# liangheming/simple_pose

Hardware: AMD Instinct MI355X
Metric: images/sec fwd+decode, ResNet50-DConv 256x192 bs=128 (higher is better)
Workload: dtype f32; 1 GPU; ResNet50-DConv 256x192 bs=128 per GPU, fp32 forward (NCHW in -> heat maps) + GaussTaylor decode, eval-mode BN, conditioned random weights; images_per_gpu=128, global_batch=128, parallelism=replicas x1 (no collective), ranks=1 process(es), one per GPU, launch=stream launches, tile_table=profiles/r06_dconv_f32_tiles.json, batches_in_flight=2, decode=in line, HSA_ENABLE_IPC_MODE_LEGACY=0

## Files before the change

### include/simple_pose_hip.h

```cpp
#ifndef SIMPLE_POSE_HIP_H
#define SIMPLE_POSE_HIP_H

#include <stdint.h>

#ifdef __cplusplus
extern "C" {
#endif

#define SP_OK 0
#define SP_EINVAL (-1)
#define SP_ELAUNCH (-2)

#define SP_ABI_VERSION 36

#define SP_CONV_RELU 0x1u
#define SP_CONV_OUT_NCHW 0x2u
#define SP_CONV_PIXEL_SHUFFLE 0x4u
#define SP_CONV_OUT_F32 0x10u
#define SP_CONV_BN_Y_MASK 0x20u
#define SP_CONV_BF16 0x8u
#define SP_CONV_HARDSWISH 0x40u
#define SP_CONV_OUT_SLICE 0x80u

typedef struct sp_conv_desc {
    int32_t batch, in_h, in_w, c_in;
    int32_t grid_h, grid_w;
    int32_t c_out;
    int32_t n_pad;
    int32_t taps_h, taps_w;
    int32_t k_pad;
    int32_t stride;
    int32_t dy0, dy_step, dx0, dx_step;
    int32_t out_h, out_w, out_c;
    int32_t oy_mul, oy_add, ox_mul, ox_add;
    int32_t phases_y, phases_x;
    uint32_t flags;
    int32_t tile_m, tile_n;
    int32_t stride_x;
    int32_t kernel;
    int32_t c_in_group;
} sp_conv_desc;

#define SP_CONV_KERNEL_IGEMM 0
#define SP_CONV_KERNEL_RING 1
#define SP_CONV_KERNEL_RING_LW 3
#define SP_CONV_KERNEL_RING_LW4 4
#define SP_CONV_KERNEL_PW 2

int sp_abi_version(void);
const char* sp_last_error(void);


int sp_nchw_to_nhwc4(const float* x_nchw, float* y_nhwc4, int batch, int channels, int h, int w, void* stream);

int sp_conv2d_fwd(const sp_conv_desc* desc, const void* x, const void* w_packed, const float* scale,
                  const float* shift, const void* residual, void* y, void* stream);

int sp_conv_set_tap_skip(int on);

int sp_conv3x3_direct_ok(const sp_conv_desc* desc);
int sp_conv3x3_direct(const sp_conv_desc* desc, const void* x, const void* w_packed, const float* scale, const float* shift,
                      const void* residual, void* y, void* stream);

int sp_basic_block_c32_ok(const sp_conv_desc* desc);
int sp_basic_block_c32(const sp_conv_desc* desc, const void* x, const void* w1_packed, const float* scale1, const float* shift1,
                       const void* w2_packed, const float* scale2, const float* shift2, void* y, void* stream);

int sp_basic_block_c64_ok(const sp_conv_desc* desc);
int sp_basic_block_c64(const sp_conv_desc* desc, const void* x, const void* w1_packed, const float* scale1, const float* shift1,
                       const void* w2_packed, const float* scale2, const float* shift2, void* y, void* stream);

int sp_dual_pw_bf16_ok(int64_t rows, int c_main, int c_short, int c_out);
int sp_dual_pw_f32_ok(int64_t rows, int c_main, int c_short, int c_out);
int sp_dual_pw_f32(const float* a_main, const float* w_main_packed, const float* scale_main, const float* shift_main, const float* a_short,
                   const float* w_short_packed, const float* scale_short, const float* shift_short, float* y, int64_t rows, int c_main, int c_short,
                   int c_out, int relu, void* stream);
int sp_dual_pw_bf16(const void* a_main, const void* w_main_packed, const float* scale_main, const float* shift_main, const void* a_short,
                    const void* w_short_packed, const float* scale_short, const float* shift_short, void* y, int64_t rows, int c_main, int c_short,
                    int c_out, int relu, void* stream);
int sp_pw_chain_f32_ok(int64_t rows, int c_mid, int c_out, int c_next);
int sp_pw_chain_f32(const float* t, const float* w3_packed, const float* scale3, const float* shift3, const float* residual, float* y,
                    const float* w1_packed, const float* scale1, const float* shift1, float* t_next, int64_t rows, int c_mid, int c_out, int c_next,
                    void* stream);
int sp_bottleneck_c64_ok(const sp_conv_desc* desc);
int sp_bottleneck_c64(const sp_conv_desc* desc, const void* x, const void* w1_packed, const float* scale1, const float* shift1,
                      const void* w2_packed, const float* scale2, const float* shift2, const void* w3_packed, const float* scale3,
                      const float* shift3, void* y, void* stream);

int sp_stem7_pool_ok(int batch, int h, int w);
int sp_stem7_pool(const float* x, const void* w_packed, int k_pad, const float* scale, const float* shift, void* y, int bf16,
                  int batch, int h, int w, void* stream);
int sp_stem7_pool_u8(const unsigned char* crops_bgr, const float* mean_rgb_host, const void* w_packed, int k_pad, const float* scale,
                     const float* shift, void* y, int bf16, int batch, int h, int w, void* stream);

int sp_hrnet_transition1_ok(int c_in, int h, int w);
int sp_hrnet_transition1(const void* x, int batch, int h, int w, const void* wa_packed, int k_pad, const float* scale_a, const float* shift_a,
                         const void* wb_packed, const float* scale_b, const float* shift_b, void* y_hi, void* y_lo, void* stream);
int sp_hrnet_stem_ok(int batch, int h, int w);
int sp_hrnet_stem(const float* x, const void* w1_packed, int k1_pad, const float* scale1, const float* shift1, const void* w2_packed,
                  const float* scale2, const float* shift2, void* y, int batch, int h, int w, void* stream);

int sp_conv2d_pw_ok(const sp_conv_desc* desc);

int sp_conv2d_ring_ok(const sp_conv_desc* desc);

int sp_conv2d_kernel_name(const sp_conv_desc* desc, int has_residual, int variant, char* buf, int cap);

int sp_conv2d_default_tile(const sp_conv_desc* desc, int* tile_m, int* tile_n);

int sp_maxpool3x3s2_nhwc(const float* x, float* y, int batch, int h, int w, int c, void* stream);

int sp_pixel_shuffle2_nhwc(const float* x, float* y, int batch, int h, int w, int c, void* stream);

int sp_global_avg_pool_nhwc(const float* x, float* y, int batch, int hw, int c, void* stream);
int sp_se_gate_add_relu_nhwc(const float* x, const float* gate_logits, const float* identity, float* y, int batch, int hw,
                             int c, void* stream);

int sp_upsample_add_nhwc(const float* x, const float* base, float* y, int batch, int h, int w, int c, int factor, int relu,
                         void* stream);
int sp_upsample_add_n_nhwc(const void* base, int bf16, int n_terms, const void* const* xs, const int32_t* factors, void* y, int batch,
                           int out_h, int out_w, int c, int relu, void* stream);

int sp_nchw_to_nhwc8_bf16(const float* x_nchw, void* y_nhwc8, int batch, int channels, int h, int w, void* stream);
int sp_maxpool3x3s2_nhwc_bf16(const void* x, void* y, int batch, int h, int w, int c, void* stream);
int sp_pixel_shuffle2_nhwc_bf16(const void* x, void* y, int batch, int h, int w, int c, void* stream);
int sp_upsample_add_nhwc_bf16(const void* x, const void* base, void* y, int batch, int h, int w, int c, int factor,
                              int relu, void* stream);
int sp_global_avg_pool_nhwc_bf16(const void* x, void* y, int batch, int hw, int c, void* stream);
int sp_se_gate_add_relu_nhwc_bf16(const void* x, const void* gate_logits, const void* identity, void* y, int batch, int hw,
                                  int c, void* stream);


int sp_heat_map_to_axis(const float* heat_nchw, int batch, int joints, int h, int w, float* coords, float* max_val,
                        void* stream);
int sp_decode_gauss_taylor(const float* heat_nchw, const float* trans_inv, int batch, int joints, int h, int w,
                           int kernel_size, float* kps, float* max_val, void* stream);
int sp_decode_basic(const float* heat_nchw, const float* trans_inv, int batch, int joints, int h, int w, float* kps,
                    float* max_val, void* stream);

int sp_heat_map_acc(const float* pred_coords, const float* label_coords, const float* mask, int batch, int joints, int h, int w,
                    float distance_thresh, float norm_frac, float* acc_out, void* stream);

int sp_u8hwc_bgr_to_nchw_f32(const unsigned char* img, float* out, int batch, int h, int w, const float* mean_rgb_host,
                             void* stream);

int sp_warp_affine_u8c3(const unsigned char* src, int src_h, int src_w, const double* m_fwd, int crops, unsigned char* dst, int out_h,
                        int out_w, void* stream);
int sp_warp_affine_batch_u8c3_to_nchw_f32(const unsigned char* const* srcs, const int* src_hw, const int* flip, const double* m_fwd, int batch,
                                          int out_h, int out_w, const float* mean_rgb_host, float* out, unsigned char* crops, void* stream);

int sp_pose_score(const float* max_val, int batch, int joints, float* score, void* stream);
int sp_pose_rescore(const float* kps, const double* box_score, int persons, int joints, double in_vis_thre, double* kps64,
                    double* score, void* stream);
int sp_oks_nms(const double* kps, const double* scores, const double* areas, const int32_t* seg, int groups, int max_group,
               int joints, const double* sigmas_host, double thresh, double vis_thresh, int32_t* keep, int32_t* keep_count,
               void* stream);

#define SP_COCO_MAX_JOINTS 64
#define SP_COCO_MAX_GT_PER_IMAGE 128
#define SP_COCO_MAX_DT_PER_IMAGE 2048
#define SP_COCO_MAX_DETS 32
#define SP_COCO_MAX_THRS 16
#define SP_COCO_MAX_AREAS 4
#define SP_COCO_MAX_REC_THRS 128
#define SP_COCO_DT_XY_F64 1
#define SP_COCO_DT_SCORE_F64 2
// ... 332 lines not shown
```

### simple_pose_amd/_lib.py

```python
from __future__ import annotations

import ctypes
import os
from ctypes import c_double, c_float, c_int, c_int32, c_int64, c_uint32, c_void_p

from .build import LIB_PATH as _DEFAULT_LIB_PATH

LIB_PATH = os.environ.get("SIMPLE_POSE_HIP_LIB", _DEFAULT_LIB_PATH)

SP_CONV_RELU = 0x1
SP_CONV_OUT_NCHW = 0x2
SP_CONV_PIXEL_SHUFFLE = 0x4
SP_CONV_BF16 = 0x8
SP_CONV_OUT_F32 = 0x10
SP_CONV_BN_Y_MASK = 0x20
SP_CONV_HARDSWISH = 0x40
SP_CONV_OUT_SLICE = 0x80
SP_LETTERBOX_FOCUS, SP_LETTERBOX_U8 = 0, 1
SP_YOLO_NMS_MAX_CANDIDATES, SP_YOLO_NMS_MAX_DET = 32768, 1024
SP_COCO_MAX_JOINTS, SP_COCO_MAX_GT_PER_IMAGE, SP_COCO_MAX_DT_PER_IMAGE, SP_COCO_MAX_DETS = 64, 128, 2048, 32
SP_COCO_DT_XY_F64, SP_COCO_DT_SCORE_F64, SP_COCO_GT_CROWD, SP_COCO_GT_IGNORE = 1, 2, 1, 2
CONV_TILES =((128, 128), (64, 128), (128, 64), (64, 64), (256, 64), (128, 32))
ABI_VERSION = 36
SP_CONV_KERNEL_IGEMM, SP_CONV_KERNEL_RING, SP_CONV_KERNEL_PW, SP_CONV_KERNEL_RING_LW, SP_CONV_KERNEL_RING_LW4 = 0, 1, 2, 3, 4
# ... 95 lines not shown
    "sp_decode_basic": (c_int, [_P, _P, c_int, c_int, c_int, c_int, _P, _P, _P]),
    "sp_heat_map_acc": (c_int, [_P, _P, _P, c_int, c_int, c_int, c_int, c_float, c_float, _P, _P]),
    "sp_u8hwc_bgr_to_nchw_f32": (c_int, [_P, _P, c_int, c_int, c_int, ctypes.POINTER(c_float), _P]),
    "sp_encode_gauss_refine": (c_int, [_P, c_int, c_int, c_int, c_int, c_float, _P, _P, _P]),
    "sp_encode_gauss_basic": (c_int, [_P, c_int, c_int, c_int, c_int, c_float, c_int, _P, _P, _P]),
    "sp_bn_train_stats_nhwc": (c_int, [_P, c_int, c_int64, c_int, c_float, c_float, _P, _P, _P, _P, _P, _P]),
    "sp_bn_apply_maxpool_nhwc": (c_int, [_P, c_int, _P, _P, _P, _P, _P, _P, c_int, c_int, c_int, c_int, _P]),
    "sp_bn_maxpool_bwd_nhwc": (c_int, [_P, c_int, _P, _P, _P, _P, _P, _P, c_int, c_int, c_int, c_int, _P, _P, _P, _P, _P]),
    "sp_bn_apply_nhwc": (c_int, [_P, c_int, _P, _P, _P, _P, _P, _P, c_int64, c_int, c_int, _P, _P]),
    "sp_bn_train_partial_nhwc": (c_int, [_P, c_int, c_int64, c_int, _P, _P, _P]),
    "sp_bn_train_finalize": (c_int, [_P, c_int64, c_int, c_float, c_float, _P, _P, _P, _P, _P]),
    "sp_bn_apply_sums_nhwc": (c_int, [_P, c_int, _P, c_int64, c_float, c_float, _P, _P, _P, _P, c_int64, c_int, c_int, _P, _P, _P, _P, _P]),
    "sp_bn_bwd_sums_from_conv2": (c_int, [_P, _P, c_int, c_int, c_int, _P, _P, _P, _P, _P]),
    "sp_bn_train_bwd_reduce_nhwc": (c_int, [_P, c_int, _P, _P, _P, _P, c_int64, c_int, _P, _P, _P, _P]),
    "sp_bn_train_bwd_apply_nhwc": (c_int, [_P, c_int, _P, _P, _P, _P, _P, _P, _P, c_int64, c_int64, c_int, _P, _P, c_int, _P]),
    "sp_bn_train_bwd_nhwc": (c_int, [_P, c_int, _P, _P, _P, _P, _P, c_int64, c_int, _P, _P, _P, _P, c_int, _P, _P]),
    "sp_channel_sum_nchw": (c_int, [_P, c_int, c_int, c_int, _P, _P]),
    "sp_channel_sum_nhwc": (c_int, [_P, c_int64, c_int, _P, _P, _P]),
    "sp_maxpool3x3s2_bwd_nhwc": (c_int, [_P, c_int, _P, _P, c_int, c_int, c_int, c_int, _P]),
    "sp_adam_step": (c_int, [_P, _P, _P, _P, c_int64, c_double, c_double, c_double, c_double, c_int, c_float, _P]),
    "sp_upsample_add_bwd_nhwc": (c_int, [_P, c_int, _P, c_int, c_int, c_int, c_int, c_int, _P, c_int, _P, c_int, _P]),
    "sp_se_gate_bwd_reduce": (c_int, [_P, c_int, _P, _P, c_int, c_int, c_int, _P, _P]),
    "sp_se_sigmoid_bwd": (c_int, [_P, c_int, _P, c_int, c_int, _P, _P, _P]),
    "sp_relu_bwd_rows": (c_int, [_P, c_int, _P, c_int, c_int, _P, _P, _P]),
    "sp_se_gate_bwd_apply": (c_int, [_P, c_int, _P, _P, _P, c_int, c_int, c_int, _P, _P, c_int, _P]),
    "sp_adam_set_scalars": (c_int, [c_double, c_double, c_double, c_double, c_int, c_float, _P, _P]),
    "sp_adam_step_dev": (c_int, [_P, _P, _P, _P, c_int64, _P, _P]),
    "sp_upsample_add_n_nhwc": (c_int, [_P, c_int, c_int, ctypes.POINTER(ctypes.c_void_p), ctypes.POINTER(c_int32), _P, c_int, c_int, c_int, c_int, c_int, _P]),
    "sp_comm_available": (c_int, []),
    "sp_comm_unique_id": (c_int, [_P]),
    "sp_comm_create": (c_int, [_P, c_int, c_int, ctypes.POINTER(ctypes.c_void_p)]),
    "sp_comm_allreduce_sum_f32": (c_int, [_P, _P, c_int64, _P]),
    "sp_comm_allreduce_sum_f64": (c_int, [_P, _P, c_int64, _P]),
    "sp_comm_info": (c_int, [_P, ctypes.POINTER(c_int), ctypes.POINTER(c_int), ctypes.POINTER(c_int)]),
    "sp_comm_destroy": (c_int, [_P]),
    "sp_conv2d_wgrad": (c_int, [ctypes.POINTER(ConvDesc), _P, c_int, _P, c_int, c_int, c_int, c_int64, c_int64, _P, _P, c_int64, _P]),
    "sp_conv2d_wgrad_workspace": (c_int, [ctypes.POINTER(WgradJob), c_int, ctypes.POINTER(c_int64)]),
    "sp_conv2d_wgrad_batched": (c_int, [ctypes.POINTER(WgradJob), c_int, _P, c_int64, _P]),
    "sp_stream_delay_us": (c_int, [c_double, _P]),
    "sp_permute4_f32": (c_int, [_P, _P, c_int, ctypes.POINTER(c_int32), ctypes.POINTER(c_int64), ctypes.POINTER(c_int32), c_int64, c_int64, _P]),
    "sp_permute4_batched": (c_int, [_P, _P, c_int, c_int, _P]),
    "sp_permute4_batched_tiled": (c_int, [_P, _P, c_int, c_int, _P]),
    "sp_pose_score": (c_int, [_P, c_int, c_int, _P, _P]),
    "sp_pose_rescore": (c_int, [_P, _P, c_int, c_int, c_double, _P, _P, _P]),
    "sp_oks_nms": (c_int, [_P, _P, _P, _P, c_int, c_int, c_int, _P, c_double, c_double, _P, _P, _P]),
    "sp_coco_kp_eval_images": (c_int, [_P, _P, _P, _P, _P, _P, _P, _P, _P, c_int, c_int, c_int, c_int, c_int, c_int, ctypes.POINTER(c_double), c_int,
                                       ctypes.POINTER(c_double), c_int, ctypes.POINTER(c_double), c_int, _P, _P, _P, _P, _P, _P, _P, _P, _P]),
    "sp_coco_kp_accumulate_workspace": (c_int, [c_int, c_int, c_int, c_int, ctypes.POINTER(c_int64)]),
    "sp_coco_kp_accumulate": (c_int, [_P, _P, _P, _P, _P, c_int, c_int, c_int, c_int, c_int, ctypes.POINTER(c_double), c_int, _P, c_int64, _P, _P, _P]),
    "sp_pixel_unshuffle2_nhwc": (c_int, [_P, _P, c_int, c_int, c_int, c_int, _P]),
    "sp_pixel_unshuffle2_nhwc_bf16": (c_int, [_P, _P, c_int, c_int, c_int, c_int, _P]),
    "sp_maxpool3x3s2_idx_nhwc": (c_int, [_P, c_int, _P, _P, c_int, c_int, c_int, c_int, _P]),
    "sp_maxpool3x3s2_bwd_idx_nhwc": (c_int, [_P, _P, c_int, _P, c_int, c_int, c_int, c_int, _P]),
    "sp_nchw_to_nhwc_pad": (c_int, [_P, _P, c_int, c_int, c_int, c_int, c_int, c_int, _P]),
    "sp_warp_affine_u8c3": (c_int, [_P, c_int, c_int, _P, c_int, _P, c_int, c_int, _P]),
    "sp_warp_affine_batch_u8c3_to_nchw_f32": (c_int, [_P, _P, _P, _P, c_int, c_int, c_int, ctypes.POINTER(c_float), _P, _P, _P]),
    "sp_conv2d_bn_stats_rows": (c_int, [ctypes.POINTER(ConvDesc), ctypes.POINTER(c_int)]),
    "sp_conv2d_fwd_bn_stats": (c_int, [ctypes.POINTER(ConvDesc), _P, _P, _P, _P, _P, c_int, _P]),
    "sp_conv2d_fwd_bn_stats_abn": (c_int, [ctypes.POINTER(ConvDesc), _P, _P, _P, _P, _P, _P, _P, _P, _P, _P, _P, c_int, _P]),
    "sp_bn_train_stats_from_conv": (c_int, [_P, _P, c_int, c_int, c_int64, c_int, c_float, c_float, _P, _P, _P, _P, _P]),
    "sp_conv2d_dgrad_bn_bwd_stats": (c_int, [ctypes.POINTER(ConvDesc), _P, _P, _P, _P, _P, _P, _P, _P, _P, _P, c_int, _P]),
    "sp_conv2d_dgrad_bn_bwd_stats2": (c_int, [ctypes.POINTER(ConvDesc), _P, _P, _P, _P, _P, _P, _P, _P, _P, _P, _P, _P, _P, _P, c_int, _P]),
    "sp_conv2d_dgrad_bn_bwd_stats_macc": (c_int, [ctypes.POINTER(ConvDesc), _P, _P, _P, _P, _P, _P, _P, _P, _P, _P, _P, _P, _P, _P, _P, c_int, _P]),
    "sp_conv2d_dgrad_phases": (c_int, [ctypes.POINTER(ConvDesc), c_int, _P, ctypes.POINTER(_P), _P, _P, _P, _P, _P, _P, _P, _P, _P, _P, _P, _P, c_int, _P]),
    "sp_bn_sums_from_conv": (c_int, [_P, _P, c_int, c_int, c_int, _P, _P]),
    "sp_bn_fold_apply_nhwc": (c_int, [_P, c_int, _P, _P, c_int, c_int, c_int64, c_float, c_float, _P, _P, _P, _P, c_int64, c_int, c_int, _P, _P, _P, _P, _P, _P]),
    "sp_bn_fold_bwd_apply_nhwc": (c_int, [_P, c_int, _P, _P, _P, _P, _P, c_int, c_int, _P, _P, _P, c_int64, c_int64, c_int, _P, _P, _P, _P, _P, _P, c_int, _P]),
    "sp_bn_bwd_sums_from_conv": (c_int, [_P, _P, c_int, c_int, c_int, _P, _P, _P]),
    "sp_bn_bwd_sums_from_conv_pair": (c_int, [_P, _P, _P, c_int, c_int, c_int, _P, _P, _P, _P, _P]),
    "sp_u8hwc_bgr_to_nhwc": (c_int, [_P, _P, c_int, c_int, c_int, c_int, _P, _P]),
    "sp_nchw_to_nhwc4_bf16": (c_int, [_P, _P, c_int, c_int, c_int, c_int, _P]),
    "sp_conv3x3_direct_ok": (c_int, [ctypes.POINTER(ConvDesc)]),
    "sp_conv3x3_direct": (c_int, [ctypes.POINTER(ConvDesc), _P, _P, _P, _P, _P, _P, _P]),
    "sp_basic_block_c32_ok": (c_int, [ctypes.POINTER(ConvDesc)]),
    "sp_basic_block_c32": (c_int, [ctypes.POINTER(ConvDesc), _P, _P, _P, _P, _P, _P, _P, _P, _P]),
    "sp_basic_block_c64_ok": (c_int, [ctypes.POINTER(ConvDesc)]),
    "sp_basic_block_c64": (c_int, [ctypes.POINTER(ConvDesc), _P, _P, _P, _P, _P, _P, _P, _P, _P]),
    "sp_dual_pw_bf16_ok": (c_int, [c_int64, c_int, c_int, c_int]),
    "sp_dual_pw_f32_ok": (c_int, [c_int64, c_int, c_int, c_int]),
    "sp_dual_pw_f32": (c_int, [_P, _P, _P, _P, _P, _P, _P, _P, _P, c_int64, c_int, c_int, c_int, c_int, _P]),
    "sp_dual_pw_bf16": (c_int, [_P, _P, _P, _P, _P, _P, _P, _P, _P, c_int64, c_int, c_int, c_int, c_int, _P]),
    "sp_pw_chain_f32_ok": (c_int, [c_int64, c_int, c_int, c_int]),
    "sp_pw_chain_f32": (c_int, [_P, _P, _P, _P, _P, _P, _P, _P, _P, _P, c_int64, c_int, c_int, c_int, _P]),
    "sp_bottleneck_c64_ok": (c_int, [ctypes.POINTER(ConvDesc)]),
    "sp_conv2d_pw_ok": (c_int, [ctypes.POINTER(ConvDesc)]),
    "sp_hrnet_stem_ok": (c_int, [c_int, c_int, c_int]),
    "sp_hrnet_stem": (c_int, [_P, _P, c_int, _P, _P, _P, _P, _P, _P, c_int, c_int, c_int, _P]),
    "sp_hrnet_transition1_ok": (c_int, [c_int, c_int, c_int]),
    "sp_hrnet_transition1": (c_int, [_P, c_int, c_int, c_int, _P, c_int, _P, _P, _P, _P, _P, _P, _P, _P]),
    "sp_stem7_pool_ok": (c_int, [c_int, c_int, c_int]),
    "sp_stem7_pool": (c_int, [_P, _P, c_int, _P, _P, _P, c_int, c_int, c_int, c_int, _P]),
    "sp_stem7_pool_u8": (c_int, [_P, ctypes.POINTER(ctypes.c_float), _P, c_int, _P, _P, _P, c_int, c_int, c_int, c_int, _P]),
    "sp_bottleneck_c64": (c_int, [ctypes.POINTER(ConvDesc), _P, _P, _P, _P, _P, _P, _P, _P, _P, _P, _P, _P]),
    "sp_masked_mse": (c_int, [_P, _P, _P, c_int, c_int, c_int, _P, _P, _P, _P]),
    "sp_conv_packed_dims": (c_int, [c_int, c_int, c_int, ctypes.POINTER(c_int), ctypes.POINTER(c_int)]),
    "sp_pack_conv_weights": (c_int, [_P, c_int, c_int, c_int, c_int, c_int, c_int, c_int, c_int, c_int, c_int, _P, c_int, _P]),
    "sp_pack_conv_weights_grouped": (c_int, [_P, c_int, c_int, c_int, c_int, c_int, _P, c_int, _P]),
    "sp_pack_conv_weights_grouped_taps": (c_int, [_P, c_int, c_int, c_int, c_int, c_int, c_int, c_int, c_int, c_int, c_int, c_int, c_int, _P, c_int, _P]),
    "sp_conv2d_wgrad_grouped_workspace": (c_int, [c_int, c_int, c_int, c_int, c_int, c_int, ctypes.POINTER(c_int64)]),
    "sp_conv2d_wgrad_grouped": (c_int, [_P, _P, c_int, c_int, c_int, c_int, c_int, c_int, c_int, c_int, c_int, c_int, c_int, c_int, _P, _P, c_int64, _P]),
    "sp_pack_deconv_k4s2p1": (c_int, [_P, c_int, c_int, c_int, _P, c_int, _P]),
    "sp_fold_bn": (c_int, [_P, _P, _P, _P, c_int, c_float, c_int, _P, _P, _P]),
    "sp_yolo_letterbox": (c_int, [_P, c_int, c_int, c_int, c_int, c_int, c_int, c_int, c_int, c_int, c_int, _P, _P]),
    "sp_yolo_focus_nchw": (c_int, [_P, c_int, c_int, c_int, _P, _P]),
    "sp_yolo_spp_nhwc": (c_int, [_P, c_int, c_int, c_int, c_int, c_int, _P]),
    "sp_upsample2_slice_nhwc": (c_int, [_P, c_int, _P, c_int, c_int, c_int, c_int, c_int, _P]),
    "sp_yolo_head_decode": (c_int, [_P, _P, _P, c_int, ctypes.POINTER(c_int32), c_int, c_int, c_int, ctypes.POINTER(c_float), ctypes.POINTER(c_float), _P, _P]),
    "sp_yolo_nms_workspace": (c_int, [c_int, ctypes.POINTER(c_int64)]),
    "sp_yolo_nms": (c_int, [_P, c_int, c_int, c_int, c_float, c_float, c_int, c_int, c_int, c_int, _P, c_int64, _P, ctypes.POINTER(c_int32), ctypes.POINTER(c_int32), _P]),
    "sp_yolo_boxes_to_source": (c_int, [_P, c_int, c_float, c_float, c_float, c_float, c_float, _P]),
    "sp_yolo_nms_device": (c_int, [_P, c_int, c_int, c_int, c_float, c_float, c_int, c_int, c_int, c_int, _P, c_int64, _P, _P, _P, _P]),
    "sp_topdown_plan": (c_int, [_P, _P, c_int, c_int, c_int, c_float, c_int, c_int, c_int, c_int, c_int, _P, _P, _P, _P, _P, _P, _P, _P, _P, _P, _P]),
    "sp_warp_affine_plan_u8c3": (c_int, [_P, c_int, c_int, c_int, _P, _P, _P, c_int, _P, c_int, c_int, _P]),
    "sp_mirror_w": (c_int, [_P, _P, c_int64, c_int, c_int, _P]),
    "sp_heat_map_flip_merge": (c_int, [_P, _P, ctypes.POINTER(c_int32), c_int, c_int, c_int, c_int, c_int, _P, _P]),
    "sp_track_associate": (c_int, [_P, _P, _P, _P, _P, _P, c_int, c_int, ctypes.POINTER(c_double), c_double, c_int, c_int, _P, _P, _P, _P, _P, _P, _P, _P,
                                   _P, _P]),
    "sp_track_boxes": (c_int, [_P, _P, _P, _P, c_int, c_int, c_float, c_float, c_float, c_int, c_int, c_int, _P, _P, _P]),
    "sp_jpeg_parse": (c_int, [_P, c_int64, ctypes.POINTER(JpegDesc), _P, c_int32]),
    "sp_jpeg_decode_batch": (c_int, [_P, _P, c_int, _P, c_int64, _P, c_int64, _P, c_int64, _P, c_int64, _P, c_int64, _P, c_int, _P]),
    "sp_jpeg_parse_scans": (c_int, [_P, c_int64, ctypes.POINTER(JpegDesc), _P, c_int32, ctypes.POINTER(c_int32), _P, c_int32]),
    "sp_jpeg_progressive_entropy": (c_int, [_P, _P, c_int, _P, _P, _P, _P, c_int64, _P, c_int64, _P, c_int64, _P, c_int64, _P, _P]),
    "sp_jpeg_enc_plan": (c_int, [c_int, c_int, c_int, c_int, c_int, ctypes.POINTER(JpegEncDesc)]),
    "sp_jpeg_encode_batch": (c_int, [_P, _P, c_int, _P, c_int64, _P, c_int64, _P, _P, c_int, _P]),
    "sp_render_workspace_bytes": (c_int, [c_int, c_int, c_int, ctypes.POINTER(c_int64)]),
    "sp_render_poses_u8c3": (c_int, [_P, _P, c_int, c_int, _P, _P, _P, _P, _P, _P, c_int, c_int, c_int, ctypes.POINTER(RenderStyle), _P, _P]),
}

_lib = None


def lib():
    global _lib
    if _lib is None:
        if not os.path.isfile(LIB_PATH):
            raise HipLibraryError(
                f"{LIB_PATH} is missing: build it with `python -m simple_pose_amd.build` (hipcc, gfx950). "
                "simple_pose_amd has no CPU/torch fallback.")
        import torch

        handle = ctypes.CDLL(LIB_PATH)
        for name, (res, args) in SYMBOLS.items():
            fn = getattr(handle, name)
            fn.restype, fn.argtypes = res, args
        if handle.sp_abi_version() != ABI_VERSION:
            raise HipLibraryError(f"ABI mismatch: library {handle.sp_abi_version()} vs binding {ABI_VERSION}")
        _lib = handle
    return _lib


def conv_kernel_name(desc, has_residual: bool = False, variant: int = 0) -> str:
    buf = ctypes.create_string_buffer(256)
    check(lib().sp_conv2d_kernel_name(desc, int(has_residual), variant, buf, 256), "sp_conv2d_kernel_name")
    return buf.value.decode()


def check(rc: int, what: str = ""):
    if rc != 0:
        msg = lib().sp_last_error().decode("utf-8", "replace")
        err = HipLibraryError(f"{what or 'libsimple_pose_hip'} failed (code {rc}): {msg}")
        err.code = rc
        raise err


def ptr(t):
    return None if t is None else t.data_ptr()
# ... 58 lines not shown
```

### simple_pose_amd/csrc/conv_pw.hip

```cpp
#include "sp_common.h"

namespace {

struct PwArgs {
    const float* x;
    const float* w;
    const float* scale;
    const float* shift;
    const float* res;
    float* y;
    int M, N, nchunks, tiles_m, relu;
    unsigned x_bytes, y_bytes;
};

constexpr int BM = 64;
constexpr int TRS = 68;
constexpr unsigned OOB = 0x80000000u;

template <int K>
__global__ __launch_bounds__(256, 1) void conv_pw_kernel(const PwArgs p) {
    constexpr int CH = K / 4;
    constexpr int NG = K / 8;
    constexpr int APT = BM * CH / 256;
    extern __shared__ __align__(16) float smem[];
// ... 353 lines not shown
        const float* a = As + cur * (BM * K);
        f32x4 fa[2][2];
#pragma unroll
        for (int i = 0; i < 2; ++i) fa[0][i] = *reinterpret_cast<const f32x4*>(a + swz(i * 32 + fr, fh));
#pragma unroll
        for (int g = 0; g < NG; ++g) {
            if (g + 1 < NG) {
#pragma unroll
                for (int i = 0; i < 2; ++i) fa[(g + 1) & 1][i] = *reinterpret_cast<const f32x4*>(a + swz(i * 32 + fr, 2 * (g + 1) + fh));
            }
#pragma unroll
            for (int s = 0; s < 4; ++s)
#pragma unroll
                for (int i = 0; i < 2; ++i)
#pragma unroll
                    for (int n = 0; n < 2; ++n)
                        acc[i][n] = __builtin_amdgcn_mfma_f32_32x32x2f32(fa[g & 1][i][s], fb[g][n][s], acc[i][n], 0, 0, 0);
        }

#pragma unroll
        for (int i = 0; i < 2; ++i)
#pragma unroll
            for (int n = 0; n < 2; ++n)
#pragma unroll
                for (int r = 0; r < 16; ++r) tr[(i * 32 + (r & 3) + 8 * (r >> 2) + 4 * fh) * TRS + n * 32 + fr] = acc[i][n][r];
#pragma unroll
        for (int it = 0; it < 16; ++it) {
            f32x4* const slot4 = reinterpret_cast<f32x4*>(tr + (it * 4 + rsub) * TRS + c4);
            f32x4 v = *slot4;
#pragma unroll
            for (int e = 0; e < 4; ++e) v[e] = v[e] * sc4[e] + sh4[e];
            const f32x4 r4 = __builtin_bit_cast(f32x4, rv[it]);
#pragma unroll
            for (int e = 0; e < 4; ++e) v[e] += r4[e];
#pragma unroll
            for (int e = 0; e < 4; ++e) v[e] = v[e] > 0.f ? v[e] : 0.f;
            __builtin_amdgcn_raw_buffer_store_b128(__builtin_bit_cast(u32x4, v), yr, off[it], 0, 0);
            *slot4 = v;
        }
        if (more) park_a(cur ^ 1);
        __syncthreads();
        if (more) load_res(mt + nslots);

        f32x16 c[RT];
#pragma unroll
        for (int i = 0; i < RT; ++i)
#pragma unroll
            for (int r = 0; r < 16; ++r) c[i][r] = 0.f;
        auto yfrag = [&](int i, int g) { return *reinterpret_cast<const f32x4*>(ys + (g >> 3) * (BM * TRS) + ((ri0 + i) * 32 + fr) * TRS + 8 * (g & 7) + 4 * fh); };
        f32x4 fy[2][RT];
#pragma unroll
        for (int i = 0; i < RT; ++i) fy[0][i] = yfrag(i, 0);
#pragma unroll
        for (int g = 0; g < NG1; ++g) {
            if (g + 1 < NG1) {
#pragma unroll
                for (int i = 0; i < RT; ++i) fy[(g + 1) & 1][i] = yfrag(i, g + 1);
            }
#pragma unroll
            for (int s = 0; s < 4; ++s)
#pragma unroll
                for (int i = 0; i < RT; ++i) c[i] = __builtin_amdgcn_mfma_f32_32x32x2f32(fy[g & 1][i][s], fw[g][s], c[i], 0, 0, 0);
        }
#pragma unroll
        for (int i = 0; i < RT; ++i)
#pragma unroll
            for (int r = 0; r < 16; ++r) {
                float v = c[i][r] * s1v + h1v;
                v = v > 0.f ? v : 0.f;
                t2[(i * 32 + (r & 3) + 8 * (r >> 2) + 4 * fh) * T2S + fr] = v;
            }
#pragma unroll
        for (int it = 0; it < RT * 4; ++it) {
            const int lr = it * 8 + (lane >> 3), cc = (lane & 7) * 4;
            const int row = m0 + ri0 * 32 + lr;
            const unsigned o = row < p.M ? (unsigned)(((size_t)row * NEXT + cn * 32 + cc) * 4) : OOB;
            const f32x4 v = *reinterpret_cast<const f32x4*>(t2 + lr * T2S + cc);
            __builtin_amdgcn_raw_buffer_store_b128(__builtin_bit_cast(u32x4, v), tnr, o, 0, 0);
        }
        __syncthreads();
    }
}

template <int NEXT>
int launch_pw_chain(const PwChainArgs& a, hipStream_t stream) {
    constexpr int lds = (2 * BM * 64 + 4 * BM * TRS + 4 * (NEXT / 64) * 32 * T2S) * 4;
    if (sp_reserve_lds<&conv_pw_chain_kernel<64, NEXT>>(lds, "conv_pw_chain")) return SP_ELAUNCH;
    int slots = sp_device_cus();
    if (slots < 1) slots = 1;
    if (slots > a.tiles_m) slots = a.tiles_m;
    const int rounds = (a.tiles_m + slots - 1) / slots;
    slots = (a.tiles_m + rounds - 1) / rounds;
    hipLaunchKernelGGL((conv_pw_chain_kernel<64, NEXT>), dim3(slots), dim3(256), lds, stream, a);
    return sp_check_launch("conv_pw_chain_kernel");
}

template <int K>
int launch_pw_dual(const PwDualArgs& a, hipStream_t stream) {
    constexpr int lds = (4 * BM * K + 4 * BM * TRS) * 4;
    if (sp_reserve_lds<&conv_pw_dual_kernel<K>>(lds, "conv_pw_dual")) return SP_ELAUNCH;
    int slots = sp_device_cus() / a.nchunks;
    if (slots < 1) slots = 1;
    if (slots > a.tiles_m) slots = a.tiles_m;
    const int rounds = (a.tiles_m + slots - 1) / slots;
    slots = (a.tiles_m + rounds - 1) / rounds;
    hipLaunchKernelGGL(conv_pw_dual_kernel<K>, dim3(slots * a.nchunks), dim3(256), lds, stream, a);
    return sp_check_launch("conv_pw_dual_kernel");
}

template <int K>
int launch_pw(const PwArgs& a, hipStream_t stream) {
    constexpr int lds = (2 * BM * K + 4 * BM * TRS) * 4;
    if (sp_reserve_lds<&conv_pw_kernel<K>>(lds, "conv_pw")) return SP_ELAUNCH;
    int slots = sp_device_cus() / a.nchunks;
    if (slots < 1) slots = 1;
    if (slots > a.tiles_m) slots = a.tiles_m;
    const int rounds = (a.tiles_m + slots - 1) / slots;
    slots = (a.tiles_m + rounds - 1) / rounds;
    hipLaunchKernelGGL(conv_pw_kernel<K>, dim3(slots * a.nchunks), dim3(256), lds, stream, a);
    return sp_check_launch("conv_pw_kernel");
}

}

extern "C" int sp_conv2d_pw_ok(const sp_conv_desc* d) {
    if (d && d->c_in_group > 0) return 0;
    if (!d) return 0;
    if (d->flags & (SP_CONV_BF16 | SP_CONV_OUT_NCHW | SP_CONV_PIXEL_SHUFFLE | SP_CONV_OUT_F32 | SP_CONV_HARDSWISH | SP_CONV_OUT_SLICE)) return 0;
    if (d->taps_h != 1 || d->taps_w != 1 || d->stride != 1 || (d->stride_x != 0 && d->stride_x != 1)) return 0;
    if (d->phases_y != 1 || d->phases_x != 1 || d->dy0 != 0 || d->dx0 != 0) return 0;
    if (d->grid_h != d->in_h || d->grid_w != d->in_w || d->out_h != d->in_h || d->out_w != d->in_w) return 0;
    if (d->oy_mul != 1 || d->ox_mul != 1 || d->oy_add != 0 || d->ox_add != 0) return 0;
    if (!(d->c_in == 64 || d->c_in == 128) || d->k_pad != d->c_in) return 0;
    if (d->c_out % 256 != 0 || d->n_pad != d->c_out || d->out_c != d->c_out) return 0;
    return 1;
}

int sp_conv_pw_launch(const sp_conv_desc* d, const void* x, const void* w_packed, const float* scale, const float* shift, const void* residual,
                      void* y, void* stream) {
    SP_REQUIRE(sp_conv2d_pw_ok(d), "sp_conv2d_fwd: kernel = SP_CONV_KERNEL_PW needs an fp32 1x1 stride-1 NHWC layer with c_in 64 / 128 and c_out %% 256 == 0");
    const long long M = (long long)d->batch * d->grid_h * d->grid_w;
    PwArgs a;
    a.x = reinterpret_cast<const float*>(x); a.w = reinterpret_cast<const float*>(w_packed); a.scale = scale; a.shift = shift;
    a.res = reinterpret_cast<const float*>(residual); a.y = reinterpret_cast<float*>(y);
    a.M = (int)M; a.N = d->c_out; a.nchunks = d->c_out / 256; a.tiles_m = (int)((M + BM - 1) / BM);
    a.relu = (d->flags & SP_CONV_RELU) ? 1 : 0;
    a.x_bytes = (unsigned)(M * d->c_in * 4); a.y_bytes = (unsigned)(M * d->c_out * 4);
    if (sp_name_query_active()) {
        sp_name_query_set("conv_pw_kernel<%d>", d->c_in);
        return SP_OK;
    }
    return d->c_in == 64 ? launch_pw<64>(a, (hipStream_t)stream) : launch_pw<128>(a, (hipStream_t)stream);
}


extern "C" int sp_dual_pw_f32_ok(int64_t rows, int c_main, int c_short, int c_out) {
    return rows > 0 && rows * (int64_t)c_out < (1ll << 30) && c_main == 64 && c_short == 64 && c_out > 0 && c_out % 256 == 0;
}

extern "C" int sp_dual_pw_f32(const float* a_main, const float* w_main_packed, const float* scale_main, const float* shift_main, const float* a_short,
                              const float* w_short_packed, const float* scale_short, const float* shift_short, float* y, int64_t rows, int c_main,
                              int c_short, int c_out, int relu, void* stream) {
    SP_REQUIRE(a_main && w_main_packed && a_short && w_short_packed && y, "sp_dual_pw_f32: null pointer");
    SP_REQUIRE(sp_dual_pw_f32_ok(rows, c_main, c_short, c_out), "sp_dual_pw_f32: two fp32 1x1 stride-1 products of 64 channels each into a multiple of 256 (got %d + %d -> %d, %lld rows)",
               c_main, c_short, c_out, (long long)rows);
    SP_REQUIRE(y != a_main && y != a_short, "sp_dual_pw_f32: y must not alias an input");
    if (sp_name_query_active()) { sp_name_query_set("conv_pw_dual_kernel<64>"); return SP_OK; }
    PwDualArgs a;
    a.x_main = a_main; a.x_short = a_short; a.w_main = w_main_packed; a.w_short = w_short_packed;
    a.s_main = scale_main; a.h_main = shift_main; a.s_short = scale_short; a.h_short = shift_short; a.y = y;
    a.M = (int)rows; a.N = c_out; a.nchunks = c_out / 256; a.tiles_m = (int)((rows + BM - 1) / BM); a.relu = relu ? 1 : 0;
    a.x_bytes = (unsigned)(rows * 64 * 4); a.y_bytes = (unsigned)(rows * c_out * 4);
    return launch_pw_dual<64>(a, (hipStream_t)stream);
}

extern "C" int sp_pw_chain_f32_ok(int64_t rows, int c_mid, int c_out, int c_next) {
    return rows > 0 && rows * (int64_t)c_out <= (1ll << 29) && c_mid == 64 && c_out == 256 && (c_next == 64 || c_next == 128);
}

extern "C" int sp_pw_chain_f32(const float* t, const float* w3_packed, const float* scale3, const float* shift3, const float* residual, float* y,
                               const float* w1_packed, const float* scale1, const float* shift1, float* t_next, int64_t rows, int c_mid, int c_out,
                               int c_next, void* stream) {
    SP_REQUIRE(t && w3_packed && residual && y && w1_packed && t_next, "sp_pw_chain_f32: null pointer");
    SP_REQUIRE(sp_pw_chain_f32_ok(rows, c_mid, c_out, c_next),
               "sp_pw_chain_f32: an fp32 1x1 product 64 -> 256 chained into a 1x1 product 256 -> 64 or 128 (got %d -> %d -> %d, %lld rows)", c_mid, c_out,
               c_next, (long long)rows);
    SP_REQUIRE(y != t && y != residual && t_next != t && t_next != residual && t_next != y, "sp_pw_chain_f32: y and t_next must not alias an input or each other");
    if (sp_name_query_active()) { sp_name_query_set("conv_pw_chain_kernel<64, %d>", c_next); return SP_OK; }
    PwChainArgs a;
    a.x = t; a.w = w3_packed; a.scale = scale3; a.shift = shift3; a.res = residual; a.y = y;
    a.w1 = w1_packed; a.scale1 = scale1; a.shift1 = shift1; a.t = t_next;
    a.M = (int)rows; a.tiles_m = (int)((rows + BM - 1) / BM);
    a.x_bytes = (unsigned)(rows * 64 * 4); a.y_bytes = (unsigned)(rows * 256 * 4); a.t_bytes = (unsigned)(rows * c_next * 4);
    return c_next == 64 ? launch_pw_chain<64>(a, (hipStream_t)stream) : launch_pw_chain<128>(a, (hipStream_t)stream);
}
```

Measured before the change: 11880 images/s.

## Add persistent software-pipelined fp32 pointwise conv kernels overlapping epilogue with MFMA

Adds persistent-block versions of the fp32 1x1 conv kernel and the dual 1x1 kernel. Each block loops over M tiles with double-buffered LDS A tiles, and interleaves the previous tile's epilogue (transpose, BN, residual, ReLU, stores) and the next tile's global loads between the MFMA instructions. The goal is to hide memory and epilogue latency behind the matrix math. The single-product pipeline is on by default (env level 1); the dual pipeline needs level 2, so it is off by default. The trade-offs are heavy register pressure, a grid sized to the CU count that may leave tiles unbalanced, and template variants specialized on residual and ReLU.

```diff
diff --git a/include/simple_pose_hip.h b/include/simple_pose_hip.h
--- a/include/simple_pose_hip.h
+++ b/include/simple_pose_hip.h
@@ -82,6 +82,7 @@
 int sp_pw_chain_f32(const float* t, const float* w3_packed, const float* scale3, const float* shift3, const float* residual, float* y,
                     const float* w1_packed, const float* scale1, const float* shift1, float* t_next, int64_t rows, int c_mid, int c_out, int c_next,
                     void* stream);
+int sp_pw_set_pipeline(int level);
 int sp_bottleneck_c64_ok(const sp_conv_desc* desc);
 int sp_bottleneck_c64(const sp_conv_desc* desc, const void* x, const void* w1_packed, const float* scale1, const float* shift1,
                       const void* w2_packed, const float* scale2, const float* shift2, const void* w3_packed, const float* scale3,
diff --git a/simple_pose_amd/_lib.py b/simple_pose_amd/_lib.py
--- a/simple_pose_amd/_lib.py
+++ b/simple_pose_amd/_lib.py
@@ -201,6 +201,7 @@
     "sp_dual_pw_bf16": (c_int, [_P, _P, _P, _P, _P, _P, _P, _P, _P, c_int64, c_int, c_int, c_int, c_int, _P]),
     "sp_pw_chain_f32_ok": (c_int, [c_int64, c_int, c_int, c_int]),
     "sp_pw_chain_f32": (c_int, [_P, _P, _P, _P, _P, _P, _P, _P, _P, _P, c_int64, c_int, c_int, c_int, _P]),
+    "sp_pw_set_pipeline": (c_int, [c_int]),
     "sp_bottleneck_c64_ok": (c_int, [ctypes.POINTER(ConvDesc)]),
     "sp_conv2d_pw_ok": (c_int, [ctypes.POINTER(ConvDesc)]),
     "sp_hrnet_stem_ok": (c_int, [c_int, c_int, c_int]),
diff --git a/simple_pose_amd/csrc/conv_pw.hip b/simple_pose_amd/csrc/conv_pw.hip
--- a/simple_pose_amd/csrc/conv_pw.hip
+++ b/simple_pose_amd/csrc/conv_pw.hip
@@ -459,6 +459,322 @@
     }
 }
 
+template <bool V>
+struct PwFlag { static constexpr bool value = V; };
+
+#define SP_PW_INLINE __attribute__((always_inline))
+
+template <int K, bool RES, bool RELU>
+__global__ __launch_bounds__(256, 1) void conv_pw_kernel(const PwArgs p) {
+    constexpr int CH = K / 4;
+    constexpr int NG = K / 8;
+    constexpr int APT = BM * CH / 256;
+    constexpr int ST = NG / 8;
+    constexpr int RD = K == 64 ? 8 : 4;
+    extern __shared__ __align__(16) float smem[];
+    float* const As = smem;
+    const int tid = threadIdx.x, lane = tid & 63, wave = tid >> 6;
+    float* const tr = smem + 2 * BM * K + wave * (BM * TRS);
+    const int fr = lane & 31, fh = lane >> 5;
+    const int nc = blockIdx.x % p.nchunks, slot0 = blockIdx.x / p.nchunks, nslots = gridDim.x / p.nchunks;
+    const int nbase = nc * 256 + wave * 64;
+
+    const __amdgpu_buffer_rsrc_t xr = __builtin_amdgcn_make_buffer_rsrc(const_cast<float*>(p.x), (short)0, p.x_bytes, 0x00020000);
+    const __amdgpu_buffer_rsrc_t yr = __builtin_amdgcn_make_buffer_rsrc(p.y, (short)0, p.y_bytes, 0x00020000);
+    const __amdgpu_buffer_rsrc_t rr = __builtin_amdgcn_make_buffer_rsrc(const_cast<float*>(RES ? p.res : p.y), (short)0, p.y_bytes, 0x00020000);
+
+    float fb[NG][2][4];
+#pragma unroll
+    for (int g = 0; g < NG; ++g)
+#pragma unroll
+        for (int n = 0; n < 2; ++n) {
+            const f32x4 t = *reinterpret_cast<const f32x4*>(p.w + (size_t)(nbase + n * 32 + fr) * K + 8 * g + 4 * fh);
+            fb[g][n][0] = t[0]; fb[g][n][1] = t[1]; fb[g][n][2] = t[2]; fb[g][n][3] = t[3];
+        }
+    const int c4 = (lane & 15) * 4, rsub = lane >> 4;
+    f32x4 sc4 = {1.f, 1.f, 1.f, 1.f}, sh4 = {0.f, 0.f, 0.f, 0.f};
+    if (p.scale) sc4 = *reinterpret_cast<const f32x4*>(p.scale + nbase + c4);
+    if (p.shift) sh4 = *reinterpret_cast<const f32x4*>(p.shift + nbase + c4);
+    const unsigned colb = (unsigned)(nbase + c4) * 4u, rowb = (unsigned)p.N * 4u;
+    const unsigned lane_off = (unsigned)rsub * rowb + colb;
+    auto voff = [&](int mt, int it) SP_PW_INLINE { return rsub < __builtin_amdgcn_readfirstlane(p.M - mt * BM - it * 4) ? lane_off : OOB; };
+    auto soff = [&](int mt, int it) SP_PW_INLINE { return __builtin_amdgcn_readfirstlane((int)((unsigned)(mt * BM + it * 4) * rowb)); };
+    float* const trw = tr + 4 * fh * TRS + fr;
+    const float* const trr = tr + rsub * TRS + c4;
+
+    auto swz = [](int row, int chunk) { return row * K + ((chunk ^ (row & (CH - 1))) << 2); };
+    constexpr int HPT = APT / 2;
+    u32x4 sa[HPT];
+    auto tile_base = [&](int mt) SP_PW_INLINE { return mt < p.tiles_m ? (unsigned)mt * (BM * K * 4) : OOB; };
+    auto load_a = [&](unsigned base, int h) SP_PW_INLINE {
+#pragma unroll
+        for (int i = 0; i < HPT; ++i) sa[i] = __builtin_amdgcn_raw_buffer_load_b128(xr, base + (unsigned)((tid + 256 * (h * HPT + i)) * 16), 0, 0);
+    };
+    auto park_a = [&](int buf, int h) SP_PW_INLINE {
+#pragma unroll
+        for (int i = 0; i < HPT; ++i) {
+            const int q = tid + 256 * (h * HPT + i);
+            *reinterpret_cast<u32x4*>(As + buf * (BM * K) + swz(q / CH, q % CH)) = sa[i];
+        }
+    };
+
+    u32x4 rv[16];
+    f32x4 pv[2];
+    auto slot = [&](auto do_epi, auto do_res, f32x16 (&e)[2][2], int j, int u, int mte, int mtg) SP_PW_INLINE {
+        if constexpr (decltype(do_epi)::value) {
+            if (u < 8) {
+                const int i = j >> 2, n = u >> 2, r = 4 * (j & 3) + (u & 3);
+                trw[(i * 32 + (r & 3) + 8 * (r >> 2)) * TRS + n * 32] = e[i][n][r];
+            } else if (u < 10) {
+                pv[u - 8] = *reinterpret_cast<const f32x4*>(trr + (2 * j + u - 8) * 4 * TRS);
+            } else if (u < 12) {
+                f32x4 v = pv[u - 10];
+#pragma unroll
+                for (int c = 0; c < 4; ++c) v[c] = v[c] * sc4[c] + sh4[c];
+                if constexpr (RES) {
+                    const f32x4 r4 = __builtin_bit_cast(f32x4, rv[2 * j + u - 10]);
+#pragma unroll
+                    for (int c = 0; c < 4; ++c) v[c] += r4[c];
+                }
+                if constexpr (RELU) {
+#pragma unroll
+                    for (int c = 0; c < 4; ++c) v[c] = v[c] > 0.f ? v[c] : 0.f;
+                }
+                pv[u - 10] = v;
+            } else if (u < 14) {
+                __builtin_amdgcn_raw_buffer_store_b128(__builtin_bit_cast(u32x4, pv[u - 12]), yr, voff(mte, 2 * j + u - 12), soff(mte, 2 * j + u - 12), 0);
+            }
+        }
+        if constexpr (RES) {
+            if (u >= 14) {
+                const int it = 2 * ((j + RD) & 7) + u - 14;
+                if (j + RD < 8) {
+                    if constexpr (decltype(do_epi)::value) rv[it] = __builtin_amdgcn_raw_buffer_load_b128(rr, voff(mte, it), soff(mte, it), 0);
+                } else {
+                    if constexpr (decltype(do_res)::value) rv[it] = __builtin_amdgcn_raw_buffer_load_b128(rr, voff(mtg, it), soff(mtg, it), 0);
+                }
+            }
+        }
+    };
+    auto gemm = [&](auto do_epi, f32x16 (&g)[2][2], f32x16 (&e)[2][2], int cur, int mtg, int mte, unsigned next) SP_PW_INLINE {
+#pragma unroll
+        for (int i = 0; i < 2; ++i)
+#pragma unroll
+            for (int n = 0; n < 2; ++n)
+#pragma unroll
+                for (int r = 0; r < 16; ++r) g[i][n][r] = 0.f;
+        const float* a = As + cur * (BM * K);
+        f32x4 fa[2][2];
+#pragma unroll
+        for (int i = 0; i < 2; ++i) fa[0][i] = *reinterpret_cast<const f32x4*>(a + swz(i * 32 + fr, fh));
+        __builtin_amdgcn_sched_barrier(0);
+#pragma unroll
+        for (int gi = 0; gi < NG; ++gi) {
+            if (gi + 1 < NG) {
+#pragma unroll
+                for (int i = 0; i < 2; ++i) fa[(gi + 1) & 1][i] = *reinterpret_cast<const f32x4*>(a + swz(i * 32 + fr, 2 * (gi + 1) + fh));
+            }
+#pragma unroll
+            for (int s = 0; s < 4; ++s)
+#pragma unroll
+                for (int i = 0; i < 2; ++i)
+#pragma unroll
+                    for (int n = 0; n < 2; ++n) {
+                        g[i][n] = __builtin_amdgcn_mfma_f32_32x32x2f32(fa[gi & 1][i][s], fb[gi][n][s], g[i][n], 0, 0, 0);
+                        const int m = gi * 16 + s * 4 + i * 2 + n;
+                        if (m % ST == 0) slot(do_epi, PwFlag<true>{}, e, (m / ST) >> 4, (m / ST) & 15, mte, mtg);
+                        if (m == 8 * NG) { park_a(cur ^ 1, 0); load_a(next, 1); }
+                        __builtin_amdgcn_sched_barrier(0);
+                    }
+        }
+    };
+    auto drain = [&](f32x16 (&e)[2][2], int mte) SP_PW_INLINE {
+#pragma unroll
+        for (int j = 0; j < 8; ++j)
+#pragma unroll
+            for (int u = 0; u < 16; ++u) slot(PwFlag<true>{}, PwFlag<false>{}, e, j, u, mte, 0);
+    };
+    auto stage = [&](auto do_epi, f32x16 (&g)[2][2], f32x16 (&e)[2][2], int cur, int mtg) SP_PW_INLINE {
+        const unsigned next = tile_base(mtg + nslots);
+        load_a(next, 0);
+        gemm(do_epi, g, e, cur, mtg, mtg - nslots, next);
+        park_a(cur ^ 1, 1);
+        __syncthreads();
+        return mtg + nslots < p.tiles_m;
+    };
+
+    int mt = slot0;
+    if (mt >= p.tiles_m) return;
+    load_a(tile_base(mt), 0);
+    park_a(0, 0);
+    load_a(tile_base(mt), 1);
+    park_a(0, 1);
+    __syncthreads();
+    f32x16 acc0[2][2], acc1[2][2];
+    bool more = stage(PwFlag<false>{}, acc0, acc1, 0, mt);
+    for (;;) {
+        if (!more) { drain(acc0, mt); break; }
+        mt += nslots;
+        more = stage(PwFlag<true>{}, acc1, acc0, 1, mt);
+        if (!more) { drain(acc1, mt); break; }
+        mt += nslots;
+        more = stage(PwFlag<true>{}, acc0, acc1, 0, mt);
+    }
+}
+
+template <int K>
+__global__ __launch_bounds__(256, 1) void conv_pw_dual_pipe_kernel(const PwDualArgs p) {
+    constexpr int CH = K / 4;
+    constexpr int NG = K / 8;
+    constexpr int APT = BM * CH / 256;
+    constexpr int ST = NG / 4;
+    extern __shared__ __align__(16) float smem[];
+    float* const As = smem;
+    const int tid = threadIdx.x, lane = tid & 63, wave = tid >> 6;
+    float* const tr = smem + 4 * BM * K + wave * (BM * TRS);
+    const int fr = lane & 31, fh = lane >> 5;
+    const int nc = blockIdx.x % p.nchunks, slot0 = blockIdx.x / p.nchunks, nslots = gridDim.x / p.nchunks;
+    const int nbase = nc * 256 + wave * 64;
+
+    const __amdgpu_buffer_rsrc_t xr0 = __builtin_amdgcn_make_buffer_rsrc(const_cast<float*>(p.x_main), (short)0, p.x_bytes, 0x00020000);
+    const __amdgpu_buffer_rsrc_t xr1 = __builtin_amdgcn_make_buffer_rsrc(const_cast<float*>(p.x_short), (short)0, p.x_bytes, 0x00020000);
+    const __amdgpu_buffer_rsrc_t yr = __builtin_amdgcn_make_buffer_rsrc(p.y, (short)0, p.y_bytes, 0x00020000);
+
+    float fb[2][NG][2][4];
+#pragma unroll
+    for (int q = 0; q < 2; ++q)
+#pragma unroll
+        for (int g = 0; g < NG; ++g)
+#pragma unroll
+            for (int n = 0; n < 2; ++n) {
+                const f32x4 t = *reinterpret_cast<const f32x4*>((q ? p.w_short : p.w_main) + (size_t)(nbase + n * 32 + fr) * K + 8 * g + 4 * fh);
+                fb[q][g][n][0] = t[0]; fb[q][g][n][1] = t[1]; fb[q][g][n][2] = t[2]; fb[q][g][n][3] = t[3];
+            }
+    float s3v[2], h3v[2], sdv[2], hdv[2];
+#pragma unroll
+    for (int n = 0; n < 2; ++n) {
+        const int ch = nbase + n * 32 + fr;
+        s3v[n] = p.s_main ? p.s_main[ch] : 1.f;  h3v[n] = p.h_main ? p.h_main[ch] : 0.f;
+        sdv[n] = p.s_short ? p.s_short[ch] : 1.f; hdv[n] = p.h_short ? p.h_short[ch] : 0.f;
+    }
+    const int c4 = (lane & 15) * 4, rsub = lane >> 4;
+    const unsigned colb = (unsigned)(nbase + c4) * 4u, rowb = (unsigned)p.N * 4u;
+    const unsigned lane_off = (unsigned)rsub * rowb + colb;
+    auto voff = [&](int mt, int it) SP_PW_INLINE { return rsub < __builtin_amdgcn_readfirstlane(p.M - mt * BM - it * 4) ? lane_off : OOB; };
+    auto soff = [&](int mt, int it) SP_PW_INLINE { return __builtin_amdgcn_readfirstlane((int)((unsigned)(mt * BM + it * 4) * rowb)); };
+    float* const trw = tr + 4 * fh * TRS + fr;
+    const float* const trr = tr + rsub * TRS + c4;
+
+    auto swz = [](int row, int chunk) { return row * K + ((chunk ^ (row & (CH - 1))) << 2); };
+    u32x4 sa[APT];
+    auto tile_base = [&](int mt) SP_PW_INLINE { return mt < p.tiles_m ? (unsigned)mt * (BM * K * 4) : OOB; };
+    auto load_a = [&](unsigned base, int q) SP_PW_INLINE {
+#pragma unroll
+        for (int i = 0; i < APT; ++i) sa[i] = __builtin_amdgcn_raw_buffer_load_b128(q ? xr1 : xr0, base + (unsigned)((tid + 256 * i) * 16), 0, 0);
+    };
+    auto park_a = [&](int buf, int q) SP_PW_INLINE {
+#pragma unroll
+        for (int i = 0; i < APT; ++i) {
+            const int e = tid + 256 * i;
+            *reinterpret_cast<u32x4*>(As + (buf * 2 + q) * (BM * K) + swz(e / CH, e % CH)) = sa[i];
+        }
+    };
+
+    f32x16 pend[2][2];
+    f32x4 pv[2];
+    auto slot = [&](int j, int u, int mte) SP_PW_INLINE {
+        if (u < 8) {
+            const int i = j >> 2, n = u >> 2, r = 4 * (j & 3) + (u & 3);
+            trw[(i * 32 + (r & 3) + 8 * (r >> 2)) * TRS + n * 32] = pend[i][n][r];
+        } else if (u < 10) {
+            pv[u - 8] = *reinterpret_cast<const f32x4*>(trr + (2 * j + u - 8) * 4 * TRS);
+        } else if (u >= 12 && u < 14) {
+            __builtin_amdgcn_raw_buffer_store_b128(__builtin_bit_cast(u32x4, pv[u - 12]), yr, voff(mte, 2 * j + u - 12), soff(mte, 2 * j + u - 12), 0);
+        }
+    };
+    auto gemm = [&](auto do_epi, int cur, int mte, unsigned next) SP_PW_INLINE {
+        f32x16 acc[2][2][2];
+#pragma unroll
+        for (int q = 0; q < 2; ++q)
+#pragma unroll
+            for (int i = 0; i < 2; ++i)
+#pragma unroll
+                for (int n = 0; n < 2; ++n)
+#pragma unroll
+                    for (int r = 0; r < 16; ++r) acc[q][i][n][r] = 0.f;
+#pragma unroll
+        for (int q = 0; q < 2; ++q) {
+            const float* a = As + (cur * 2 + q) * (BM * K);
+            f32x4 fa[2][2];
+#pragma unroll
+            for (int i = 0; i < 2; ++i) fa[0][i] = *reinterpret_cast<const f32x4*>(a + swz(i * 32 + fr, fh));
+            __builtin_amdgcn_sched_barrier(0);
+#pragma unroll
+            for (int gi = 0; gi < NG; ++gi) {
+                if (gi + 1 < NG) {
+#pragma unroll
+                    for (int i = 0; i < 2; ++i) fa[(gi + 1) & 1][i] = *reinterpret_cast<const f32x4*>(a + swz(i * 32 + fr, 2 * (gi + 1) + fh));
+                }
+#pragma unroll
+                for (int s = 0; s < 4; ++s)
+#pragma unroll
+                    for (int i = 0; i < 2; ++i)
+#pragma unroll
+                        for (int n = 0; n < 2; ++n) {
+                            acc[q][i][n] = __builtin_amdgcn_mfma_f32_32x32x2f32(fa[gi & 1][i][s], fb[q][gi][n][s], acc[q][i][n], 0, 0, 0);
+                            if constexpr (decltype(do_epi)::value) {
+                                const int m = (q * NG + gi) * 16 + s * 4 + i * 2 + n;
+                                if (m % ST == 0) slot((m / ST) >> 4, (m / ST) & 15, mte);
+                            }
+                            if (q == 1 && gi == 0 && s == 0 && i == 0 && n == 1) { park_a(cur ^ 1, 0); load_a(next, 1); }
+                            __builtin_amdgcn_sched_barrier(0);
+                        }
+            }
+        }
+#pragma unroll
+        for (int i = 0; i < 2; ++i)
+#pragma unroll
+            for (int n = 0; n < 2; ++n)
+#pragma unroll
+                for (int r = 0; r < 16; ++r) {
+                    const float vd = acc[1][i][n][r] * sdv[n] + hdv[n];
+                    float v = acc[0][i][n][r] * s3v[n] + h3v[n];
+                    v += vd;
+                    if (p.relu) v = v > 0.f ? v : 0.f;
+                    pend[i][n][r] = v;
+                }
+    };
+    auto stage = [&](auto do_epi, int cur, int mtg) SP_PW_INLINE {
+        const unsigned next = tile_base(mtg + nslots);
+        load_a(next, 0);
+        gemm(do_epi, cur, mtg - nslots, next);
+        park_a(cur ^ 1, 1);
+        __syncthreads();
+        return mtg + nslots < p.tiles_m;
+    };
+
+    int mt = slot0;
+    if (mt >= p.tiles_m) return;
+    load_a(tile_base(mt), 0);
+    park_a(0, 0);
+    load_a(tile_base(mt), 1);
+    park_a(0, 1);
+    __syncthreads();
+    bool more = stage(PwFlag<false>{}, 0, mt);
+    for (;;) {
+        if (!more) break;
+        mt += nslots;
+        more = stage(PwFlag<true>{}, 1, mt);
+        if (!more) break;
+        mt += nslots;
+        more = stage(PwFlag<true>{}, 0, mt);
+    }
+#pragma unroll
+    for (int j = 0; j < 8; ++j)
+#pragma unroll
+        for (int u = 0; u < 14; ++u) slot(j, u, mt);
+}
+
 template <int NEXT>
 int launch_pw_chain(const PwChainArgs& a, hipStream_t stream) {
     constexpr int lds = (2 * BM * 64 + 4 * BM * TRS + 4 * (NEXT / 64) * 32 * T2S) * 4;
@@ -498,6 +814,53 @@
     return sp_check_launch("conv_pw_kernel");
 }
 
+template <int K>
+int launch_pw_dual_pipe(const PwDualArgs& a, hipStream_t stream) {
+    constexpr int lds = (4 * BM * K + 4 * BM * TRS) * 4;
+    if (sp_reserve_lds<&conv_pw_dual_pipe_kernel<K>>(lds, "conv_pw_dual_pipe")) return SP_ELAUNCH;
+    int slots = sp_device_cus() / a.nchunks;
+    if (slots < 1) slots = 1;
+    if (slots > a.tiles_m) slots = a.tiles_m;
+    const int rounds = (a.tiles_m + slots - 1) / slots;
+    slots = (a.tiles_m + rounds - 1) / rounds;
+    hipLaunchKernelGGL((conv_pw_dual_pipe_kernel<K>), dim3(slots * a.nchunks), dim3(256), lds, stream, a);
+    return sp_check_launch("conv_pw_dual_pipe_kernel");
+}
+
+template <int K, bool RES, bool RELU>
+int launch_pw_pipe(const PwArgs& a, hipStream_t stream) {
+    constexpr int lds = (2 * BM * K + 4 * BM * TRS) * 4;
+    if (sp_reserve_lds<&conv_pw_kernel<K, RES, RELU>>(lds, "conv_pw_pipe")) return SP_ELAUNCH;
+    int slots = sp_device_cus() / a.nchunks;
+    if (slots < 1) slots = 1;
+    if (slots > a.tiles_m) slots = a.tiles_m;
+    const int rounds = (a.tiles_m + slots - 1) / slots;
+    slots = (a.tiles_m + rounds - 1) / rounds;
+    hipLaunchKernelGGL((conv_pw_kernel<K, RES, RELU>), dim3(slots * a.nchunks), dim3(256), lds, stream, a);
+    return sp_check_launch("conv_pw_kernel (pipelined)");
+}
+
+template <int K>
+int launch_pw_pipe_flags(const PwArgs& a, hipStream_t stream) {
+    if (a.res) return a.relu ? launch_pw_pipe<K, true, true>(a, stream) : launch_pw_pipe<K, true, false>(a, stream);
+    return a.relu ? launch_pw_pipe<K, false, true>(a, stream) : launch_pw_pipe<K, false, false>(a, stream);
+}
+
+int g_pw_pipeline = -1;
+int pw_pipeline_level() {
+    if (g_pw_pipeline < 0) {
+        const char* e = getenv("SP_PW_PIPELINE");
+        const int v = e ? atoi(e) : 1;
+        g_pw_pipeline = v < 0 ? 0 : v > 2 ? 2 : v;
+    }
+    return g_pw_pipeline;
+}
+
+}
+
+extern "C" int sp_pw_set_pipeline(int level) {
+    g_pw_pipeline = level < 0 ? 0 : level > 2 ? 2 : level;
+    return SP_OK;
 }
 
 extern "C" int sp_conv2d_pw_ok(const sp_conv_desc* d) {
@@ -523,10 +886,13 @@
     a.M = (int)M; a.N = d->c_out; a.nchunks = d->c_out / 256; a.tiles_m = (int)((M + BM - 1) / BM);
     a.relu = (d->flags & SP_CONV_RELU) ? 1 : 0;
     a.x_bytes = (unsigned)(M * d->c_in * 4); a.y_bytes = (unsigned)(M * d->c_out * 4);
+    const bool pipe = pw_pipeline_level() >= 1 && a.y_bytes <= OOB && a.x_bytes <= OOB;
     if (sp_name_query_active()) {
-        sp_name_query_set("conv_pw_kernel<%d>", d->c_in);
+        if (pipe) sp_name_query_set("conv_pw_kernel<%d, %s, %s>", d->c_in, a.res ? "true" : "false", a.relu ? "true" : "false");
+        else sp_name_query_set("conv_pw_kernel<%d>", d->c_in);
         return SP_OK;
     }
+    if (pipe) return d->c_in == 64 ? launch_pw_pipe_flags<64>(a, (hipStream_t)stream) : launch_pw_pipe_flags<128>(a, (hipStream_t)stream);
     return d->c_in == 64 ? launch_pw<64>(a, (hipStream_t)stream) : launch_pw<128>(a, (hipStream_t)stream);
 }
 
@@ -542,12 +908,18 @@
     SP_REQUIRE(sp_dual_pw_f32_ok(rows, c_main, c_short, c_out), "sp_dual_pw_f32: two fp32 1x1 stride-1 products of 64 channels each into a multiple of 256 (got %d + %d -> %d, %lld rows)",
                c_main, c_short, c_out, (long long)rows);
     SP_REQUIRE(y != a_main && y != a_short, "sp_dual_pw_f32: y must not alias an input");
-    if (sp_name_query_active()) { sp_name_query_set("conv_pw_dual_kernel<64>"); return SP_OK; }
+    const bool pipe = pw_pipeline_level() >= 2 && rows * c_out * 4 <= (int64_t)OOB;
+    if (sp_name_query_active()) {
+        if (pipe) sp_name_query_set("conv_pw_dual_pipe_kernel<64>");
+        else sp_name_query_set("conv_pw_dual_kernel<64>");
+        return SP_OK;
+    }
     PwDualArgs a;
     a.x_main = a_main; a.x_short = a_short; a.w_main = w_main_packed; a.w_short = w_short_packed;
     a.s_main = scale_main; a.h_main = shift_main; a.s_short = scale_short; a.h_short = shift_short; a.y = y;
     a.M = (int)rows; a.N = c_out; a.nchunks = c_out / 256; a.tiles_m = (int)((rows + BM - 1) / BM); a.relu = relu ? 1 : 0;
     a.x_bytes = (unsigned)(rows * 64 * 4); a.y_bytes = (unsigned)(rows * c_out * 4);
+    if (pipe) return launch_pw_dual_pipe<64>(a, (hipStream_t)stream);
     return launch_pw_dual<64>(a, (hipStream_t)stream);
 }
 
```

Result: no change. 11990 images/s (median of 6 runs) (+0.9%).
